# xander683/ConstructionScenePoseEstimation

Measured on AMD Instinct MI355X. Metric: annotated frames/sec (RGB+seg+2D kpts) at 1920×1080, 1/2/4/8 MI355X, higher is better.
Workload: dtype f32

## Files before the change

constructionsceneposeestimation_amd/csrc/csg_kernels.hip:

```cpp
#include <math.h>

#include <algorithm>

#include <type_traits>

#include "csg_crops.h"
#include "csg_kernels.h"
#include "csg_raster_math.h"

namespace csg {

#ifndef CSG_ABLATION
#define CSG_ABLATION 0
#endif
#define DBG(d) (CSG_ABLATION ? (d) : 0u)

constexpr uint64_t kEmptyKey = ~0ull;

__device__ __forceinline__ uint32_t fbits(float f) { return __float_as_uint(f); }

template <int Ctrl, int RowMask, int BankMask>
__device__ __forceinline__ uint32_t dpp_add(uint32_t v) {
  return v + (uint32_t)__builtin_amdgcn_update_dpp(0, (int)v, Ctrl, RowMask, BankMask, false);
}
// ... 891 lines not shown
        } else {
          for (uint32_t d = (ex2 >> 5) + 1u; d <= (e_end >> 5); ++d) L.before[d] = (uint16_t)(ci + 1u);
        }
      }
      __syncthreads();
      for (uint32_t j = tid; j < ((DBG(b.dbg) & 8u) ? 0u : tot2); j += kRB) {
        if (DBG(b.dbg) & 512u) {
          const uint64_t m = __ballot(1);
          if ((uint32_t)__lane_id() == (uint32_t)__ffsll((unsigned long long)m) - 1u) {
            atomicAdd(&b.overflow[14], 1u);
            atomicAdd(&b.overflow[15], (uint32_t)__popcll(m));
          }
        }
        const uint32_t w = L.starts[j >> 5], nb = L.before[j >> 5];
        const uint32_t rank = nb + (uint32_t)__popc(w & (0xFFFFFFFFu >> (31u - (j & 31u))));
        const uint32_t spj = L.span[rank - 1u];
        fragment<kCov>(c, L.img, (int)(spj & 255u), (int)(j + (uint32_t)kTileW - (spj >> 16)), (int)((spj >> 8) & 255u));
      }
      __syncthreads();
    }
  }
}

struct ShadeEntry {
  float P[16];
  int32_t label;
  int32_t tex;
  uint32_t base;
  uint32_t q01, q2;
  uint32_t n01, n2;
};

__device__ __forceinline__ void shade_setup(const SceneDev& s, const BatchDev& b, uint32_t f, uint32_t uid,
                                            ShadeEntry& e) {
  const uint32_t i = uid >> s.uid_shift, g = uid & ((1u << s.uid_shift) - 1u);
  const uint32_t set = b.fset[f];
  const float* tp = s.tri_pos + (size_t)g * 9;
  float p[9];
#pragma unroll
  for (int z = 0; z < 9; ++z) p[z] = tp[z];
  const InstSetDev is = b.iset[(size_t)set * s.n_inst + i];
  e.label = is.label;
  const int tex = is.tex;
  e.tex = tex;
  e.base = is.base;
  const float* tu = s.tri_uv + (size_t)g * 6;
#pragma unroll
  for (int z = 0; z < 6; ++z) e.P[10 + z] = tex >= 0 ? tu[z] : 0.0f;
  bool facing = false;
  if (tex >= 0 || b.depth || b.points || b.normals) {
    Cv3 v[3];
    const float* Cm = b.clip + ((size_t)f * s.n_inst + i) * 12;
#pragma unroll
    for (int z = 0; z < 3; ++z) {
      v[z].x = dot4(Cm + 0, p[3 * z], p[3 * z + 1], p[3 * z + 2]);
      v[z].y = dot4(Cm + 4, p[3 * z], p[3 * z + 1], p[3 * z + 2]);
      v[z].w = dot4(Cm + 8, p[3 * z], p[3 * z + 1], p[3 * z + 2]);
    }
    Hom h;
    hom_setup(v, h);
#pragma unroll
    for (int z = 0; z < 3; ++z) { e.P[z] = h.A[z]; e.P[3 + z] = h.B[z]; e.P[6 + z] = h.C[z]; }
    e.P[9] = h.invdet;
    facing = h.invdet < 0.0f;
  }
  float e1[3], e2[3];
  {
    const float* M = b.models + ((size_t)set * s.n_inst + i) * 16;
#pragma unroll
    for (int r = 0; r < 3; ++r) {
      const float w0 = dot4(M + 4 * r, p[0], p[1], p[2]);
      const float w1 = dot4(M + 4 * r, p[3], p[4], p[5]);
      const float w2 = dot4(M + 4 * r, p[6], p[7], p[8]);
      e1[r] = w1 - w0;
      e2[r] = w2 - w0;
    }
  }
  const float nx = e1[1] * e2[2] - e1[2] * e2[1];
  const float ny = e1[2] * e2[0] - e1[0] * e2[2];
  const float nz = e1[0] * e2[1] - e1[1] * e2[0];
  const float nn = (nx * nx + ny * ny) + nz * nz;
  const LightDev& L = b.lights[set];
  float cs = 0.0f;
  uint32_t n01 = 0, n2 = 0;
  if (nn > 0.0f) {
    const float len = sqrtf(nn);
    const float d = (nx * L.sun_dir[0] + ny * L.sun_dir[1]) + nz * L.sun_dir[2];
    cs = fabsf(d / len);
    if (b.normals) {
      const float sg = facing ? 1.0f : -1.0f;
      n01 = half_bits(sg * (nx / len)) | (half_bits(sg * (ny / len)) << 16);
      n2 = half_bits(sg * (nz / len));
    }
  }
  e.n01 = n01;
  e.n2 = n2;
  uint32_t q[3];
#pragma unroll
  for (int z = 0; z < 3; ++z) {
    const float shade = L.ambient[z] + L.sun[z] * cs;
    const int qq = (int)(shade * 256.0f + 0.5f);
    q[z] = (uint32_t)min(max(qq, 0), 65535);
  }
  e.q01 = q[0] | (q[1] << 16);
  e.q2 = q[2];
  __asm__ volatile("" ::: "memory");
  float P[16];
#pragma unroll
  for (int z = 0; z < 16; ++z) P[z] = e.P[z];
  float D[3], U[3], V[3];
  depth_plane(P, P + 3, P + 6, P[9], D);
  uv_planes(P, P + 3, P + 6, P[9], P + 10, U, V);
#pragma unroll
  for (int z = 0; z < 3; ++z) { e.P[z] = D[z]; e.P[4 + 2 * z] = U[z]; e.P[5 + 2 * z] = V[z]; }
}

__device__ __forceinline__ void shade_pixel(const SceneDev& s, const ShadeEntry& e, int px, int py, bool need_depth,
                                            uint32_t& rgb_out, int32_t& id_out, float& depth_out) {
  const bool textured = e.tex >= 0 && !(DBG(s.dbg) & 4096u);
  const float fx = (float)px + 0.5f, fy = (float)py + 0.5f;
  float r = INFINITY;
  if (need_depth || textured) r = rcp_ieee(plane_at(e.P[0], e.P[1], e.P[2], fx, fy));
  depth_out = need_depth ? r : INFINITY;
  id_out = e.label;
  int base[3] = {(int)(e.base & 255u), (int)((e.base >> 8) & 255u), (int)((e.base >> 16) & 255u)};
  int alb[3];
  if (textured) {
    const f32x2 p0 = {e.P[4], e.P[5]}, p1 = {e.P[6], e.P[7]}, p2 = {e.P[8], e.P[9]};
    const f32x2 uv = ((p0 * fx + p1 * fy) + p2) * r;
    int c[4];
    tex_sample(s, e.tex, uv.x, uv.y, c);
#pragma unroll
    for (int z = 0; z < 3; ++z) alb[z] = div255(__umul24((uint32_t)c[z], (uint32_t)base[z]) + 127u);
  } else {
#pragma unroll
    for (int z = 0; z < 3; ++z) alb[z] = base[z];
  }
  const int q[3] = {(int)(e.q01 & 0xFFFFu), (int)(e.q01 >> 16), (int)e.q2};
  uint32_t o = 0;
#pragma unroll
  for (int z = 0; z < 3; ++z) o |= (uint32_t)min((int)((__umul24((uint32_t)alb[z], (uint32_t)q[z]) + 128u) >> 8), 255) << (8 * z);
  rgb_out = o;
}

#ifndef CSG_VEC_OUT
#define CSG_VEC_OUT 1
#endif
#ifndef CSG_VEC_DEP_ONCE
#define CSG_VEC_DEP_ONCE 1
#endif

#ifndef CSG_SHADE_SLOTS
#define CSG_SHADE_SLOTS (kRasterBlock >= 256 ? 116 : 64)
#endif
constexpr uint32_t kShadeSlots = CSG_SHADE_SLOTS;
static_assert(kShadeSlots <= (uint32_t)kRasterBlock && kShadeSlots < 255u, "one setup thread per slot; 8-bit slot ids");
constexpr int kShadeProbes = 16;
struct ResolveLds {
  uint32_t keys[kShadeSlots];
  uint32_t more;
  ShadeEntry tab[kShadeSlots];
  uint32_t lstat[2 + kColWords][kMaxLdsLabels];
};

constexpr size_t lds_budget(int waves) {
  return kRasterBlock == 256
             ? (waves >= 8 ? 20480u : waves == 7 ? 22528u : waves == 6 ? 26700u : waves == 5 ? 32256u : 40960u)
             : ((157696u / (size_t)(waves * 4 / (kRasterBlock / 64))) & ~511u);
}
static_assert((sizeof(RasterLds<kStage>) > sizeof(ResolveLds) ? sizeof(RasterLds<kStage>) : sizeof(ResolveLds)) +
                      kTilePix * 8 <= lds_budget(CSG_WAVES),
              "k_raster LDS must allow CSG_WAVES workgroups per CU");

template <bool kCov>
struct RasterSide {
  RasterLds<kStageOf<kCov>> r;
};
template <>
struct RasterSide<true> {
  RasterLds<kStageOf<true>> r;
  CovLds cov;
  int32_t rlabel[kStageOf<true>];
};
static_assert((sizeof(RasterSide<true>) > sizeof(ResolveLds) ? sizeof(RasterSide<true>) : sizeof(ResolveLds)) +
                      kTilePix * 8 <= lds_budget(CSG_COV_WAVES),
              "k_raster<true> LDS must allow CSG_COV_WAVES workgroups per CU");

__device__ __forceinline__ int shade_slot(uint32_t* keys, uint32_t uid) {
  const uint32_t h = __umulhi(uid * 2654435761u, kShadeSlots);
#pragma clang loop vectorize(disable) unroll(disable)
  for (int p = 0; p < kShadeProbes; ++p) {
    uint32_t idx = h + (uint32_t)p;
    idx = idx >= kShadeSlots ? idx - kShadeSlots : idx;
    const uint32_t prev = atomicCAS(&keys[idx], kNoAlpha, uid);
    if (prev == kNoAlpha || prev == uid) return (int)idx;
  }
  return -1;
}

#ifndef CSG_SQ_X
#define CSG_SQ_X 2
#endif
#ifndef CSG_SQ_Y
#define CSG_SQ_Y 2
#endif
constexpr uint32_t kSqX = CSG_SQ_X, kSqY = CSG_SQ_Y;
constexpr uint32_t kSqN = kSqX * kSqY;
// ... 17 lines not shown
#endif
#ifndef CSG_NT_RGB
#define CSG_NT_RGB 1
#endif
typedef uint32_t v3u32 __attribute__((ext_vector_type(3)));
typedef float v4f32 __attribute__((ext_vector_type(4)));
typedef uint32_t v2u32 __attribute__((ext_vector_type(2)));
__device__ __forceinline__ void out_f4(float* p, float a, float b2, float c, float d) {
  const v4f32 w = {a, b2, c, d};
  if (CSG_NT_OUT) __builtin_nontemporal_store(w, reinterpret_cast<v4f32*>(p));
  else *reinterpret_cast<v4f32*>(p) = w;
}
__device__ __forceinline__ void out_u2(uint16_t* p, uint32_t a, uint32_t b2) {
  const v2u32 w = {a, b2};
  if (CSG_NT_OUT) __builtin_nontemporal_store(w, reinterpret_cast<v2u32*>(p));
  else *reinterpret_cast<v2u32*>(p) = w;
}
__device__ __forceinline__ void out_rgb4(uint8_t* p, uint32_t c0, uint32_t c1, uint32_t c2, uint32_t c3) {
  const v3u32 w = {c0 | (c1 << 24), (c1 >> 8) | (c2 << 16), (c2 >> 16) | (c3 << 8)};
  if (CSG_NT_RGB) __builtin_nontemporal_store(w, reinterpret_cast<v3u32*>(p));
  else *reinterpret_cast<v3u32*>(p) = w;
}

__device__ __forceinline__ void empty_tile(const SceneDev& s, const BatchDev& b, uint32_t f, uint32_t tile, int ox,
                                           int oy) {
  const int tid = threadIdx.x;
  if (b.n_kp && ((b.kp_tiles[(size_t)f * b.tile_words + (tile >> 5)] >> (tile & 31u)) & 1u)) {
    for (uint32_t k = tid; k < b.n_kp; k += kRB) {
      const size_t o = (size_t)f * b.n_kp + k;
      const uint32_t pp = b.kp_pix[o];
      const int px = (int)(pp & 0xFFFFu) - ox, py = (int)(pp >> 16) - oy;
      if (pp == 0xFFFFFFFFu || px < 0 || px >= kTileW || py < 0 || py >= kTileH) continue;
      b.kp_vis[o] = (b.kp_w[o] <= INFINITY) ? 2 : 1;
    }
  }
  const int ly = tid / (kTileW / 4), lx0 = (tid % (kTileW / 4)) * 4;
  const int py = oy + ly, px0 = ox + lx0;
  if (py >= (int)s.H) return;
  const size_t o = (size_t)f * s.W * s.H + (size_t)py * s.W + px0;
  const uint32_t sky = b.lights[b.fset[f]].sky & 0xFFFFFFu;
  const float nan = __builtin_nanf("");
  if (px0 + 3 < (int)s.W && ((o + b.px_align) & 3u) == 0) {
    if (b.inst) out_ids(b.inst + o, make_int4(-1, -1, -1, -1));
    if (b.rgb) out_rgb4(b.rgb + o * 3, sky, sky, sky, sky);
    if (b.depth) out_f4(b.depth + o, INFINITY, INFINITY, INFINITY, INFINITY);
    if (b.normals) {
      for (int w = 0; w < 3; ++w) out_u2(b.normals + o * 3 + 4 * w, 0u, 0u);
    }
    if (b.points) {
      for (int w = 0; w < 3; ++w) out_f4(b.points + o * 3 + 4 * w, nan, nan, nan, nan);
    }
  } else {
    for (int k = 0; k < 4 && px0 + k < (int)s.W; ++k) {
      if (b.inst) b.inst[o + k] = -1;
      if (b.rgb) {
        b.rgb[(o + k) * 3 + 0] = (uint8_t)(sky & 255u);
        b.rgb[(o + k) * 3 + 1] = (uint8_t)((sky >> 8) & 255u);
        b.rgb[(o + k) * 3 + 2] = (uint8_t)((sky >> 16) & 255u);
      }
      if (b.depth) b.depth[o + k] = INFINITY;
      if (b.normals) b.normals[(o + k) * 3 + 0] = b.normals[(o + k) * 3 + 1] = b.normals[(o + k) * 3 + 2] = 0;
      if (b.points) b.points[(o + k) * 3 + 0] = b.points[(o + k) * 3 + 1] = b.points[(o + k) * 3 + 2] = nan;
    }
  }
}

template <bool kCov>
__global__ __launch_bounds__(kRasterBlock) CSG_RASTER_ATTR void k_raster(SceneDev s, BatchDev b) {
  __shared__ unsigned long long zb[kTilePix];
  constexpr int NS = kStageOf<kCov>;
  __shared__ union Lds {
    RasterSide<kCov> ra;
    ResolveLds q;
  } L;
  const int tid = threadIdx.x;
  uint32_t tile;
  if (!swizzled_tile(blockIdx.x, s.tiles_x, s.tiles_y, tile)) return;
  const uint32_t f = blockIdx.y;
  const int ox = (int)(tile % s.tiles_x) * kTileW, oy = (int)(tile / s.tiles_x) * kTileH;
  const uint32_t* toff = b.tile_off + (size_t)f * (s.n_tiles + 1);
  const Slab sb = b.slab[f];
  const uint32_t beg = min(toff[tile], sb.bin_cap);
  const uint32_t end = (DBG(b.dbg) & 2u) ? beg : min(toff[tile + 1], sb.bin_cap);
  if (beg == end && !(DBG(b.dbg) & 2u)) {
    empty_tile(s, b, f, tile, ox, oy);
    return;
  }
  const uint32_t* bins = b.bins + sb.bin_base;
  const uint32_t rfirst = (CSG_PREFETCH_BIN && tid < NS && beg + (uint32_t)tid < end) ? bins[beg + tid] : 0xFFFFFFFFu;
  for (int p = tid; p < kTilePix; p += kRB) zb[p] = kEmptyKey;
  CovLds* covp = nullptr;
  int32_t* rlabel = nullptr;
  if constexpr (kCov) {
    covp = &L.ra.cov;
    rlabel = L.ra.rlabel;
    CovLds& covl = *covp;
    for (int p = tid; p < kCovSlots * (kTilePix / 32); p += kRB) (&covl.mask[0][0])[p] = 0u;
    if (tid < kCovSlots) covl.keys[tid] = kNoAlpha;
    if (tid == 0) covl.ovf = 0u;
  }
  const Rec* recs = b.recs + sb.rec_base;
  RasterCtx c{s.aquad, s.acls, zb, ox, oy, s.inv_near, s.inv_far, b.dbg, b.overflow, covp, rlabel,
              kCov ? b.covered + (size_t)f * b.n_labels : nullptr};
  __syncthreads();
  raster_block<kCov, NS>(c, s, b, L.ra.r, beg, end, bins, recs, sb.rec_cap, rfirst);
  __syncthreads();
  if constexpr (kCov) {
    const CovLds& covl = *covp;
// ... 9 lines not shown
    if ((tid % kTPS) == 0 && lab != kNoAlpha) {
      if (covl.ovf) atomicOr(&c.gcov[lab], kCovUnknown);
      else atomicAdd(&c.gcov[lab], n);
    }
    __syncthreads();
  }

  if (DBG(b.dbg) & 1u) {
    if (tid == 0 && zb[0] == 0ull && b.inst) b.inst[0] = 0;
    return;
  }
  if (b.n_kp && ((b.kp_tiles[(size_t)f * b.tile_words + (tile >> 5)] >> (tile & 31u)) & 1u)) {
    for (uint32_t k = tid; k < b.n_kp; k += kRB) {
      const size_t o = (size_t)f * b.n_kp + k;
      const uint32_t pp = b.kp_pix[o];
      const int px = (int)(pp & 0xFFFFu) - ox, py = (int)(pp >> 16) - oy;
      if (pp == 0xFFFFFFFFu || px < 0 || px >= kTileW || py < 0 || py >= kTileH) continue;
      const unsigned long long key = zb[zb_index(px, py)];
      const float d = key == kEmptyKey ? INFINITY : rcp_ieee(__uint_as_float(0xFFFFFFFFu - (uint32_t)(key >> 32)));
      b.kp_vis[o] = (b.kp_w[o] <= d) ? 2 : 1;
    }
    __syncthreads();
  }
  const bool want_stats = b.stats != nullptr;
  const uint32_t nl = want_stats ? min(b.n_labels, (uint32_t)kMaxLdsLabels) : 0u;
  uint32_t (*lstat)[kMaxLdsLabels] = L.q.lstat;
  for (uint32_t l = tid; l < nl; l += kRB) {
#pragma unroll
    for (int w = 0; w < 2 + kColWords; ++w) lstat[w][l] = 0;
  }
  const int ly = tid / (kTileW / 4), lx0 = (tid % (kTileW / 4)) * 4;
  const int py = oy + ly;
  const bool row_ok = py < (int)s.H;
  const int px0 = ox + lx0;
  unsigned long long* zrow = &zb[zb_index(lx0, ly) & ~3];
  const int zsw = CSG_ZB_SWIZZLE ? (ly & 3) : 0;
  auto zpix = [&](int k) -> unsigned long long& { return zrow[k ^ zsw]; };
  uint32_t pend = 0;
  uint32_t inmask = 0;
  __shared__ uint32_t drw[2][kRB / 64];
  {
    const uint32_t sky = b.lights[b.fset[f]].sky & 0xFFFFFFu;
    const unsigned long long bgword = (unsigned long long)sky | (0xFFFFFFFFull << 32);
    uint32_t kmn = 0xFFFFFFFFu, kmx = 0u;
#pragma unroll
    for (int k = 0; k < 4; ++k) {
      const bool in = row_ok && px0 + k < (int)s.W;
      inmask |= in ? 1u << k : 0u;
      const unsigned long long key = zpix(k);
      if (in && key != kEmptyKey) {
        pend |= 1u << k;
        kmn = min(kmn, (uint32_t)(key >> 32));
        kmx = max(kmx, (uint32_t)(key >> 32));
      } else {
        zpix(k) = bgword;
      }
    }
    if (b.drange) {
#pragma unroll
      for (int o = 32; o > 0; o >>= 1) {
        kmn = min(kmn, (uint32_t)__shfl_xor((int)kmn, o, 64));
        kmx = max(kmx, (uint32_t)__shfl_xor((int)kmx, o, 64));
      }
      if ((tid & 63) == 0) { drw[0][tid >> 6] = kmn; drw[1][tid >> 6] = kmx; }
    }
  }
  const size_t npx = (size_t)s.W * s.H;
  const size_t o = (size_t)f * npx + (size_t)py * s.W + px0;
  const uint32_t bgmask = inmask & ~pend;
  const bool need_depth = b.depth || b.points;
  auto round = [&](const bool first) __attribute__((always_inline)) -> bool {
    if ((uint32_t)tid < kShadeSlots) L.q.keys[tid] = kNoAlpha;
    __syncthreads();
    if (tid == 0) L.q.more = 0;
    if (first && b.drange && tid == 0) {
      uint32_t kmn = drw[0][0], kmx = drw[1][0];
#pragma unroll
      for (int w = 1; w < kRB / 64; ++w) { kmn = min(kmn, drw[0][w]); kmx = max(kmx, drw[1][w]); }
      if (kmn <= kmx) {
        const float dmin = rcp_ieee(__uint_as_float(0xFFFFFFFFu - kmn));
        const float dmax = rcp_ieee(__uint_as_float(0xFFFFFFFFu - kmx));
        if (__float_as_uint(dmin) < b.drange[f]) atomicMin(&b.drange[f], __float_as_uint(dmin));
        if (__float_as_uint(dmax) > b.drange[b.drange_F + f]) atomicMax(&b.drange[b.drange_F + f], __float_as_uint(dmax));
      }
    }
    uint32_t slots = 0xFFFFFFFFu;
    {
      uint32_t prev_uid = 0xFFFFFFFFu, prev_slot = 0xFFu;
#pragma unroll
      for (int k = 0; k < 4; ++k) {
        if ((pend >> k) & 1u) {
          const uint32_t uid = (uint32_t)zpix(k);
          uint32_t sl;
          if (uid == prev_uid) sl = prev_slot;
          else {
            const int r = shade_slot(L.q.keys, uid);
            sl = r < 0 ? 0xFFu : (uint32_t)r;
          }
          prev_uid = uid;
          prev_slot = sl;
          slots = (slots & ~(0xFFu << (8 * k))) | (sl << (8 * k));
        } else {
          prev_uid = 0xFFFFFFFFu;
        }
      }
    }
    __syncthreads();
    {
      const uint32_t u = (uint32_t)tid < kShadeSlots ? L.q.keys[tid] : kNoAlpha;
      if (u != kNoAlpha) {
        ShadeEntry& e = L.q.tab[tid];
        if (DBG(b.dbg) & 8192u) {
          e = ShadeEntry{};
          e.P[2] = 1.0f; e.tex = -1; e.label = 0;
        } else {
          shade_setup(s, b, f, u, e);
        }
      }
    }
    __syncthreads();
    if (row_ok) {
      int qx0 = px0, qy = py;
      asm volatile("" : "+v"(qx0), "+v"(qy));
      const size_t qo = (size_t)f * npx + (size_t)qy * s.W + qx0;
      int32_t run = -1;
      uint32_t cnt = 0, xmin = 0, xmax = 0;
      auto flush_run = [&]() {
        if (DBG(b.dbg) & 16384u) return;
        if (run >= 0 && (uint32_t)run < nl) {
          const uint32_t col = xmin - (uint32_t)ox;
          atomicAdd(&lstat[0][run], cnt);
          atomicOr(&lstat[2 + (kColWords > 1 ? col >> 5 : 0u)][run], (0xFu >> (3u - (xmax - xmin))) << (col & 31u));
          atomicOr(&lstat[1][run], 1u << ((uint32_t)qy - (uint32_t)oy));
        } else if (run >= 0 && b.stats && (uint32_t)run < b.n_labels) {
          uint32_t* st = b.stats + ((size_t)f * b.n_labels + (uint32_t)run) * 5;
          atomicAdd(&st[0], cnt);
          atomicMin(&st[1], xmin);
          atomicMin(&st[2], (uint32_t)qy);
          atomicMax(&st[3], xmax);
          atomicMax(&st[4], (uint32_t)qy);
        }
      };
      bool vec = false;
      if (CSG_VEC_OUT && (b.depth || b.normals || b.points) && inmask == 0xFu && ((qo + b.px_align) & 3u) == 0) {
        uint32_t done = first ? bgmask : 0u;
#pragma unroll
        for (int k = 0; k < 4; ++k) done |= ((slots >> (8 * k)) & 0xFFu) != 0xFFu ? 1u << k : 0u;
        vec = done == 0xFu;
      }
#pragma unroll
      for (int k = 0; k < 4; ++k) {
        const int px = qx0 + k;
        const uint32_t sl = (slots >> (8 * k)) & 0xFFu;
        const bool bg = first && ((bgmask >> k) & 1u);
        if (sl == 0xFFu && !bg) continue;
        float dep = INFINITY;
        uint32_t n01 = 0, n2 = 0;
        if (!bg) {
          const ShadeEntry& e = L.q.tab[sl];
          uint32_t rgb;
          int32_t id;
          shade_pixel(s, e, px, qy, need_depth && !(CSG_VEC_DEP_ONCE && vec), rgb, id, dep);
          n01 = e.n01;
          n2 = e.n2;
          zpix(k) = (unsigned long long)rgb | ((unsigned long long)(uint32_t)id << 32);
          pend &= ~(1u << k);
          if (want_stats) {
            if (id != run) {
              flush_run();
              run = id;
              cnt = 0;
              xmin = (uint32_t)px;
            }
            ++cnt;
            xmax = (uint32_t)px;
          }
        }
        if (vec) continue;
        if (b.depth) b.depth[qo + k] = dep;
        if (b.normals) {
          uint16_t* d = b.normals + (qo + k) * 3;
          d[0] = (uint16_t)(n01 & 0xFFFFu);
          d[1] = (uint16_t)(n01 >> 16);
          d[2] = (uint16_t)n2;
        }
        if (b.points) {
          float pt[3];
          if (bg) pt[0] = pt[1] = pt[2] = __builtin_nanf("");
          else unproject(b.cam + (size_t)f * kCamFloats, px, qy, dep, pt);
          float* d = b.points + (qo + k) * 3;
          d[0] = pt[0];
          d[1] = pt[1];
          d[2] = pt[2];
        }
      }
      flush_run();
      if (vec) {
        const uint32_t bgv = first ? bgmask : 0u;
        float dv[4];
#pragma unroll
        for (int k = 0; k < 4; ++k) {
          const ShadeEntry& e = L.q.tab[(bgv >> k) & 1u ? 0u : (slots >> (8 * k)) & 0xFFu];
          const float fx = (float)(qx0 + k) + 0.5f, fy = (float)qy + 0.5f;
          dv[k] = ((bgv >> k) & 1u) || !need_depth ? INFINITY : rcp_ieee(plane_at(e.P[0], e.P[1], e.P[2], fx, fy));
        }
        if (b.depth) out_f4(b.depth + qo, dv[0], dv[1], dv[2], dv[3]);
        if (b.normals) {
          uint32_t n01[4], n2[4];
#pragma unroll
          for (int k = 0; k < 4; ++k) {
            const bool bg = (bgv >> k) & 1u;
            const ShadeEntry& e = L.q.tab[bg ? 0u : (slots >> (8 * k)) & 0xFFu];
            n01[k] = bg ? 0u : e.n01;
            n2[k] = bg ? 0u : e.n2;
          }
          uint16_t* d = b.normals + qo * 3;
          out_u2(d, n01[0], n2[0] | (n01[1] << 16));
          out_u2(d + 4, (n01[1] >> 16) | (n2[1] << 16), n01[2]);
          out_u2(d + 8, n2[2] | (n01[3] << 16), (n01[3] >> 16) | (n2[3] << 16));
        }
        if (b.points) {
          float pt[12];
#pragma unroll
          for (int k = 0; k < 4; ++k) {
            if ((bgv >> k) & 1u) pt[3 * k] = pt[3 * k + 1] = pt[3 * k + 2] = __builtin_nanf("");
            else unproject(b.cam + (size_t)f * kCamFloats, qx0 + k, qy, dv[k], pt + 3 * k);
          }
          float* d = b.points + qo * 3;
          out_f4(d, pt[0], pt[1], pt[2], pt[3]);
          out_f4(d + 4, pt[4], pt[5], pt[6], pt[7]);
          out_f4(d + 8, pt[8], pt[9], pt[10], pt[11]);
        }
      }
    }
    if (pend) L.q.more = 1;
    __syncthreads();
    return L.q.more != 0;
  };
  if (round(true)) {
#pragma clang loop unroll(disable)
    while (round(false)) {
    }
  }
  if (row_ok) {
    uint32_t rgb[4];
    int32_t ids[4];
#pragma unroll
    for (int k = 0; k < 4; ++k) {
      const unsigned long long w = zpix(k);
      rgb[k] = (uint32_t)w;
      ids[k] = (int32_t)(w >> 32);
    }
    if (px0 + 3 < (int)s.W && ((o + b.px_align) & 3u) == 0) {
      if (b.inst) out_ids(b.inst + o, make_int4(ids[0], ids[1], ids[2], ids[3]));
      if (b.rgb) out_rgb4(b.rgb + o * 3, rgb[0], rgb[1], rgb[2], rgb[3]);
    } else {
      for (int k = 0; k < 4 && px0 + k < (int)s.W; ++k) {
        if (b.inst) b.inst[o + k] = ids[k];
        if (b.rgb) {
          b.rgb[(o + k) * 3 + 0] = (uint8_t)(rgb[k] & 255u);
          b.rgb[(o + k) * 3 + 1] = (uint8_t)((rgb[k] >> 8) & 255u);
          b.rgb[(o + k) * 3 + 2] = (uint8_t)((rgb[k] >> 16) & 255u);
        }
      }
    }
  }
  if (b.stats) {
    __syncthreads();
    uint32_t* st = b.stats + (size_t)f * b.n_labels * 5;
    for (uint32_t l = tid; l < nl; l += kRB) {
      const uint32_t cnt = lstat[0][l];
      if (cnt) {
        const uint32_t rm = lstat[1][l];
        uint32_t cm = lstat[2][l], cm_hi = cm, lo_w = 0, hi_w = 0;
#pragma unroll
        for (int w = 1; w < kColWords; ++w) {
          const uint32_t m = lstat[2 + w][l];
          if (!cm && m) { cm = m; lo_w = (uint32_t)w; }
          if (m) { cm_hi = m; hi_w = (uint32_t)w; }
        }
        if (!cm_hi) cm_hi = cm;
        atomicAdd(&st[l * 5 + 0], cnt);
        atomicMin(&st[l * 5 + 1], (uint32_t)ox + 32u * lo_w + (uint32_t)(__ffs(cm) - 1));
        atomicMin(&st[l * 5 + 2], (uint32_t)oy + (uint32_t)(__ffs(rm) - 1));
        atomicMax(&st[l * 5 + 3], (uint32_t)ox + 32u * hi_w + 31u - (uint32_t)__clz(cm_hi));
        atomicMax(&st[l * 5 + 4], (uint32_t)oy + 31u - (uint32_t)__clz(rm));
      }
    }
  }
}

__global__ void k_init_stats(uint32_t* st, uint32_t n) {
  const uint32_t k = blockIdx.x * blockDim.x + threadIdx.x;
  if (k < n) {
    const uint32_t c = k % 5;
    st[k] = (c == 1 || c == 2) ? 0xFFFFFFFFu : 0u;
  }
}

__device__ __forceinline__ void project_one(const float* pv, const float* p, float Wf, float Hf, float nearc,
                                            float& u, float& v, int& vis, int& px, int& py) {
  const float X = dot4(pv + 0, p[0], p[1], p[2]);
  const float Y = dot4(pv + 4, p[0], p[1], p[2]);
  const float Wc = dot4(pv + 8, p[0], p[1], p[2]);
  px = py = -1;
  if (!(Wc >= nearc)) {
    u = -1.0f; v = -1.0f; vis = 0;
    return;
  }
// ... 227 lines not shown
                 uint64_t bin_pool, int use_hints, Slab* slab, uint64_t* need, hipStream_t st) {
  hipLaunchKernelGGL(k_plan, dim3(1), dim3(64), 0, st, frames, F, def_rec, def_bin, rec_pool, bin_pool, use_hints,
                     slab, need);
}

void launch_scan(const SceneDev& s, const BatchDev& b, uint32_t F, hipStream_t st) {
  hipLaunchKernelGGL(k_scan, dim3(F), dim3(kBlock), 0, st, s, b);
}

void launch_bin(const SceneDev& s, const BatchDev& b, uint32_t F, uint32_t blocks, hipStream_t st) {
  dim3 g(blocks, F);
  const uint32_t band = s.n_tiles < kBinBand ? s.n_tiles : kBinBand;
  if (s.n_tiles > kBinBand) hipLaunchKernelGGL(k_bin<true>, g, dim3(kBlock), band * sizeof(uint32_t), st, s, b);
  else hipLaunchKernelGGL(k_bin<false>, g, dim3(kBlock), band * sizeof(uint32_t), st, s, b);
}

void launch_colscan(const SceneDev& s, const BatchDev& b, uint32_t F, hipStream_t st) {
  hipLaunchKernelGGL(k_colscan, dim3((s.n_tiles + kBlock - 1) / kBlock, F), dim3(kBlock), 0, st, s, b);
}

void launch_raster(const SceneDev& s, const BatchDev& b, uint32_t F, hipStream_t st) {
  const uint32_t squares = ((s.tiles_x + kSqX - 1) / kSqX) * ((s.tiles_y + kSqY - 1) / kSqY);
  dim3 g(8 * kSqN * ((squares + 7) / 8), F);
  if (b.covered) hipLaunchKernelGGL(k_raster<true>, g, dim3(kRasterBlock), 0, st, s, b);
  else hipLaunchKernelGGL(k_raster<false>, g, dim3(kRasterBlock), 0, st, s, b);
}

void launch_init_stats(const BatchDev& b, uint32_t F, hipStream_t st) {
  const uint32_t n = F * b.n_labels * 5;
  if (!n || !b.stats) return;
  hipLaunchKernelGGL(k_init_stats, dim3((n + 255) / 256), dim3(256), 0, st, b.stats, n);
}

void launch_keypoints(const SceneDev& s, const BatchDev& b, uint32_t F, hipStream_t st) {
  if (!b.n_kp) return;
  dim3 g((b.n_kp + 255) / 256, F);
  hipLaunchKernelGGL(k_keypoints, g, dim3(256), 0, st, s, b);
}

void launch_inst_bounds(const SceneDev& s, const Chunk* chunks, uint32_t n_chunks, const float* models,
                        uint32_t* out, hipStream_t st) {
  hipLaunchKernelGGL(k_inst_bounds, dim3(n_chunks), dim3(kBlock), 0, st, s, chunks, models, out);
}

void launch_project(const float* pts, uint32_t n, const float* pv12, float W, float H, float near_clip, float* uv,
                    int32_t* vis, hipStream_t st) {
  hipLaunchKernelGGL(k_project, dim3((n + 255) / 256), dim3(256), 0, st, pts, n, pv12, W, H, near_clip, uv, vis);
}
// ... 269 lines not shown
```

Baseline: 25750.

## Add lean raster kernel specialization for RGB+seg-only outputs

Adds a compile-time kLean variant of k_raster that is chosen when depth, normals, points, stats and drange are all disabled. The variant removes normal and depth plane handling, label-stat LDS tables and depth-range reductions, and shrinks the shade entry and resolve LDS. It also recomputes per-thread pixel coordinates from tid at several points, so fewer values stay live in registers and occupancy can rise. The cost is a third kernel instantiation, more code to maintain, and a little extra index arithmetic.

```diff
diff --git a/constructionsceneposeestimation_amd/csrc/csg_kernels.hip b/constructionsceneposeestimation_amd/csrc/csg_kernels.hip
--- a/constructionsceneposeestimation_amd/csrc/csg_kernels.hip
+++ b/constructionsceneposeestimation_amd/csrc/csg_kernels.hip
@@ -937,6 +937,7 @@
   }
 }
 
+template <bool kLean>
 struct ShadeEntry {
   float P[16];
   int32_t label;
@@ -945,9 +946,24 @@
   uint32_t q01, q2;
   uint32_t n01, n2;
 };
-
+template <>
+struct ShadeEntry<true> {
+  float P[16];
+  int32_t label;
+  int32_t tex;
+  uint32_t base;
+  uint32_t q01, q2;
+};
+template <bool kLean>
+struct SetupOpt {
+  bool facing = false;
+};
+template <>
+struct SetupOpt<true> {};
+
+template <bool kLean>
 __device__ __forceinline__ void shade_setup(const SceneDev& s, const BatchDev& b, uint32_t f, uint32_t uid,
-                                            ShadeEntry& e) {
+                                            ShadeEntry<kLean>& e) {
   const uint32_t i = uid >> s.uid_shift, g = uid & ((1u << s.uid_shift) - 1u);
   const uint32_t set = b.fset[f];
   const float* tp = s.tri_pos + (size_t)g * 9;
@@ -962,8 +978,8 @@
   const float* tu = s.tri_uv + (size_t)g * 6;
 #pragma unroll
   for (int z = 0; z < 6; ++z) e.P[10 + z] = tex >= 0 ? tu[z] : 0.0f;
-  bool facing = false;
-  if (tex >= 0 || b.depth || b.points || b.normals) {
+  SetupOpt<kLean> opt;
+  if (tex >= 0 || (!kLean && (b.depth || b.points || b.normals))) {
     Cv3 v[3];
     const float* Cm = b.clip + ((size_t)f * s.n_inst + i) * 12;
 #pragma unroll
@@ -977,7 +993,7 @@
 #pragma unroll
     for (int z = 0; z < 3; ++z) { e.P[z] = h.A[z]; e.P[3 + z] = h.B[z]; e.P[6 + z] = h.C[z]; }
     e.P[9] = h.invdet;
-    facing = h.invdet < 0.0f;
+    if constexpr (!kLean) opt.facing = h.invdet < 0.0f;
   }
   float e1[3], e2[3];
   {
@@ -997,19 +1013,27 @@
   const float nn = (nx * nx + ny * ny) + nz * nz;
   const LightDev& L = b.lights[set];
   float cs = 0.0f;
-  uint32_t n01 = 0, n2 = 0;
-  if (nn > 0.0f) {
-    const float len = sqrtf(nn);
-    const float d = (nx * L.sun_dir[0] + ny * L.sun_dir[1]) + nz * L.sun_dir[2];
-    cs = fabsf(d / len);
-    if (b.normals) {
-      const float sg = facing ? 1.0f : -1.0f;
-      n01 = half_bits(sg * (nx / len)) | (half_bits(sg * (ny / len)) << 16);
-      n2 = half_bits(sg * (nz / len));
-    }
-  }
-  e.n01 = n01;
-  e.n2 = n2;
+  if constexpr (kLean) {
+    if (nn > 0.0f) {
+      const float len = sqrtf(nn);
+      const float d = (nx * L.sun_dir[0] + ny * L.sun_dir[1]) + nz * L.sun_dir[2];
+      cs = fabsf(d / len);
+    }
+  } else {
+    uint32_t n01 = 0, n2 = 0;
+    if (nn > 0.0f) {
+      const float len = sqrtf(nn);
+      const float d = (nx * L.sun_dir[0] + ny * L.sun_dir[1]) + nz * L.sun_dir[2];
+      cs = fabsf(d / len);
+      if (b.normals) {
+        const float sg = opt.facing ? 1.0f : -1.0f;
+        n01 = half_bits(sg * (nx / len)) | (half_bits(sg * (ny / len)) << 16);
+        n2 = half_bits(sg * (nz / len));
+      }
+    }
+    e.n01 = n01;
+    e.n2 = n2;
+  }
   uint32_t q[3];
 #pragma unroll
   for (int z = 0; z < 3; ++z) {
@@ -1030,13 +1054,18 @@
   for (int z = 0; z < 3; ++z) { e.P[z] = D[z]; e.P[4 + 2 * z] = U[z]; e.P[5 + 2 * z] = V[z]; }
 }
 
-__device__ __forceinline__ void shade_pixel(const SceneDev& s, const ShadeEntry& e, int px, int py, bool need_depth,
-                                            uint32_t& rgb_out, int32_t& id_out, float& depth_out) {
+template <bool kLean>
+__device__ __forceinline__ void shade_pixel(const SceneDev& s, const ShadeEntry<kLean>& e, int px, int py,
+                                            bool need_depth, uint32_t& rgb_out, int32_t& id_out, float& depth_out) {
   const bool textured = e.tex >= 0 && !(DBG(s.dbg) & 4096u);
   const float fx = (float)px + 0.5f, fy = (float)py + 0.5f;
   float r = INFINITY;
-  if (need_depth || textured) r = rcp_ieee(plane_at(e.P[0], e.P[1], e.P[2], fx, fy));
-  depth_out = need_depth ? r : INFINITY;
+  if constexpr (kLean) {
+    if (textured) r = rcp_ieee(plane_at(e.P[0], e.P[1], e.P[2], fx, fy));
+  } else {
+    if (need_depth || textured) r = rcp_ieee(plane_at(e.P[0], e.P[1], e.P[2], fx, fy));
+    depth_out = need_depth ? r : INFINITY;
+  }
   id_out = e.label;
   int base[3] = {(int)(e.base & 255u), (int)((e.base >> 8) & 255u), (int)((e.base >> 16) & 255u)};
   int alb[3];
@@ -1071,11 +1100,18 @@
 constexpr uint32_t kShadeSlots = CSG_SHADE_SLOTS;
 static_assert(kShadeSlots <= (uint32_t)kRasterBlock && kShadeSlots < 255u, "one setup thread per slot; 8-bit slot ids");
 constexpr int kShadeProbes = 16;
+template <bool kLean>
 struct ResolveLds {
   uint32_t keys[kShadeSlots];
   uint32_t more;
-  ShadeEntry tab[kShadeSlots];
+  ShadeEntry<false> tab[kShadeSlots];
   uint32_t lstat[2 + kColWords][kMaxLdsLabels];
+};
+template <>
+struct ResolveLds<true> {
+  uint32_t keys[kShadeSlots];
+  uint32_t more;
+  ShadeEntry<true> tab[kShadeSlots];
 };
 
 constexpr size_t lds_budget(int waves) {
@@ -1083,7 +1119,7 @@
              ? (waves >= 8 ? 20480u : waves == 7 ? 22528u : waves == 6 ? 26700u : waves == 5 ? 32256u : 40960u)
              : ((157696u / (size_t)(waves * 4 / (kRasterBlock / 64))) & ~511u);
 }
-static_assert((sizeof(RasterLds<kStage>) > sizeof(ResolveLds) ? sizeof(RasterLds<kStage>) : sizeof(ResolveLds)) +
+static_assert((sizeof(RasterLds<kStage>) > sizeof(ResolveLds<false>) ? sizeof(RasterLds<kStage>) : sizeof(ResolveLds<false>)) +
                       kTilePix * 8 <= lds_budget(CSG_WAVES),
               "k_raster LDS must allow CSG_WAVES workgroups per CU");
 
@@ -1097,7 +1133,7 @@
   CovLds cov;
   int32_t rlabel[kStageOf<true>];
 };
-static_assert((sizeof(RasterSide<true>) > sizeof(ResolveLds) ? sizeof(RasterSide<true>) : sizeof(ResolveLds)) +
+static_assert((sizeof(RasterSide<true>) > sizeof(ResolveLds<false>) ? sizeof(RasterSide<true>) : sizeof(ResolveLds<false>)) +
                       kTilePix * 8 <= lds_budget(CSG_COV_WAVES),
               "k_raster<true> LDS must allow CSG_COV_WAVES workgroups per CU");
 
@@ -1161,6 +1197,7 @@
   else *reinterpret_cast<v3u32*>(p) = w;
 }
 
+template <bool kLean>
 __device__ __forceinline__ void empty_tile(const SceneDev& s, const BatchDev& b, uint32_t f, uint32_t tile, int ox,
                                            int oy) {
   const int tid = threadIdx.x;
@@ -1178,16 +1215,18 @@
   if (py >= (int)s.H) return;
   const size_t o = (size_t)f * s.W * s.H + (size_t)py * s.W + px0;
   const uint32_t sky = b.lights[b.fset[f]].sky & 0xFFFFFFu;
-  const float nan = __builtin_nanf("");
+  [[maybe_unused]] const float nan = __builtin_nanf("");
   if (px0 + 3 < (int)s.W && ((o + b.px_align) & 3u) == 0) {
     if (b.inst) out_ids(b.inst + o, make_int4(-1, -1, -1, -1));
     if (b.rgb) out_rgb4(b.rgb + o * 3, sky, sky, sky, sky);
-    if (b.depth) out_f4(b.depth + o, INFINITY, INFINITY, INFINITY, INFINITY);
-    if (b.normals) {
-      for (int w = 0; w < 3; ++w) out_u2(b.normals + o * 3 + 4 * w, 0u, 0u);
-    }
-    if (b.points) {
-      for (int w = 0; w < 3; ++w) out_f4(b.points + o * 3 + 4 * w, nan, nan, nan, nan);
+    if constexpr (!kLean) {
+      if (b.depth) out_f4(b.depth + o, INFINITY, INFINITY, INFINITY, INFINITY);
+      if (b.normals) {
+        for (int w = 0; w < 3; ++w) out_u2(b.normals + o * 3 + 4 * w, 0u, 0u);
+      }
+      if (b.points) {
+        for (int w = 0; w < 3; ++w) out_f4(b.points + o * 3 + 4 * w, nan, nan, nan, nan);
+      }
     }
   } else {
     for (int k = 0; k < 4 && px0 + k < (int)s.W; ++k) {
@@ -1197,20 +1236,40 @@
         b.rgb[(o + k) * 3 + 1] = (uint8_t)((sky >> 8) & 255u);
         b.rgb[(o + k) * 3 + 2] = (uint8_t)((sky >> 16) & 255u);
       }
-      if (b.depth) b.depth[o + k] = INFINITY;
-      if (b.normals) b.normals[(o + k) * 3 + 0] = b.normals[(o + k) * 3 + 1] = b.normals[(o + k) * 3 + 2] = 0;
-      if (b.points) b.points[(o + k) * 3 + 0] = b.points[(o + k) * 3 + 1] = b.points[(o + k) * 3 + 2] = nan;
-    }
-  }
-}
-
-template <bool kCov>
+      if constexpr (!kLean) {
+        if (b.depth) b.depth[o + k] = INFINITY;
+        if (b.normals) b.normals[(o + k) * 3 + 0] = b.normals[(o + k) * 3 + 1] = b.normals[(o + k) * 3 + 2] = 0;
+        if (b.points) b.points[(o + k) * 3 + 0] = b.points[(o + k) * 3 + 1] = b.points[(o + k) * 3 + 2] = nan;
+      }
+    }
+  }
+}
+
+__device__ __forceinline__ uint32_t (*drange_lds())[kRasterBlock / 64] {
+  __shared__ uint32_t drw[2][kRasterBlock / 64];
+  return drw;
+}
+template <bool kLean>
+struct ResolveOpt {
+  bool want_stats, need_depth;
+  uint32_t nl;
+  uint32_t (*lstat)[kMaxLdsLabels];
+  uint32_t (*drw)[kRasterBlock / 64];
+};
+template <>
+struct ResolveOpt<true> {};
+
+#ifndef CSG_RASTER_LEAN
+#define CSG_RASTER_LEAN 1
+#endif
+template <bool kCov, bool kLean>
 __global__ __launch_bounds__(kRasterBlock) CSG_RASTER_ATTR void k_raster(SceneDev s, BatchDev b) {
+  static_assert(!(kCov && kLean), "the coverage kernel is general");
   __shared__ unsigned long long zb[kTilePix];
   constexpr int NS = kStageOf<kCov>;
   __shared__ union Lds {
     RasterSide<kCov> ra;
-    ResolveLds q;
+    ResolveLds<kLean> q;
   } L;
   const int tid = threadIdx.x;
   uint32_t tile;
@@ -1222,7 +1281,7 @@
   const uint32_t beg = min(toff[tile], sb.bin_cap);
   const uint32_t end = (DBG(b.dbg) & 2u) ? beg : min(toff[tile + 1], sb.bin_cap);
   if (beg == end && !(DBG(b.dbg) & 2u)) {
-    empty_tile(s, b, f, tile, ox, oy);
+    empty_tile<kLean>(s, b, f, tile, ox, oy);
     return;
   }
   const uint32_t* bins = b.bins + sb.bin_base;
@@ -1278,27 +1337,39 @@
     }
     __syncthreads();
   }
-  const bool want_stats = b.stats != nullptr;
-  const uint32_t nl = want_stats ? min(b.n_labels, (uint32_t)kMaxLdsLabels) : 0u;
-  uint32_t (*lstat)[kMaxLdsLabels] = L.q.lstat;
-  for (uint32_t l = tid; l < nl; l += kRB) {
-#pragma unroll
-    for (int w = 0; w < 2 + kColWords; ++w) lstat[w][l] = 0;
+  ResolveOpt<kLean> opt;
+  if constexpr (!kLean) {
+    opt.want_stats = b.stats != nullptr;
+    opt.nl = opt.want_stats ? min(b.n_labels, (uint32_t)kMaxLdsLabels) : 0u;
+    opt.lstat = L.q.lstat;
+    opt.drw = drange_lds();
+    for (uint32_t l = tid; l < opt.nl; l += kRB) {
+#pragma unroll
+      for (int w = 0; w < 2 + kColWords; ++w) opt.lstat[w][l] = 0;
+    }
   }
   const int ly = tid / (kTileW / 4), lx0 = (tid % (kTileW / 4)) * 4;
   const int py = oy + ly;
   const bool row_ok = py < (int)s.H;
   const int px0 = ox + lx0;
   unsigned long long* zrow = &zb[zb_index(lx0, ly) & ~3];
-  const int zsw = CSG_ZB_SWIZZLE ? (ly & 3) : 0;
+  int zsw = CSG_ZB_SWIZZLE ? (ly & 3) : 0;
   auto zpix = [&](int k) -> unsigned long long& { return zrow[k ^ zsw]; };
+  auto zfresh = [&]() __attribute__((always_inline)) {
+    if constexpr (kLean) {
+      int t = tid;
+      asm volatile("" : "+v"(t));
+      const int y = t / (kTileW / 4), x0 = (t % (kTileW / 4)) * 4;
+      zrow = &zb[zb_index(x0, y) & ~3];
+      zsw = CSG_ZB_SWIZZLE ? (y & 3) : 0;
+    }
+  };
   uint32_t pend = 0;
   uint32_t inmask = 0;
-  __shared__ uint32_t drw[2][kRB / 64];
   {
     const uint32_t sky = b.lights[b.fset[f]].sky & 0xFFFFFFu;
     const unsigned long long bgword = (unsigned long long)sky | (0xFFFFFFFFull << 32);
-    uint32_t kmn = 0xFFFFFFFFu, kmx = 0u;
+    [[maybe_unused]] uint32_t kmn = 0xFFFFFFFFu, kmx = 0u;
 #pragma unroll
     for (int k = 0; k < 4; ++k) {
       const bool in = row_ok && px0 + k < (int)s.W;
@@ -1306,41 +1377,48 @@
       const unsigned long long key = zpix(k);
       if (in && key != kEmptyKey) {
         pend |= 1u << k;
-        kmn = min(kmn, (uint32_t)(key >> 32));
-        kmx = max(kmx, (uint32_t)(key >> 32));
+        if constexpr (!kLean) {
+          kmn = min(kmn, (uint32_t)(key >> 32));
+          kmx = max(kmx, (uint32_t)(key >> 32));
+        }
       } else {
         zpix(k) = bgword;
       }
     }
-    if (b.drange) {
-#pragma unroll
-      for (int o = 32; o > 0; o >>= 1) {
-        kmn = min(kmn, (uint32_t)__shfl_xor((int)kmn, o, 64));
-        kmx = max(kmx, (uint32_t)__shfl_xor((int)kmx, o, 64));
-      }
-      if ((tid & 63) == 0) { drw[0][tid >> 6] = kmn; drw[1][tid >> 6] = kmx; }
+    if constexpr (!kLean) {
+      if (b.drange) {
+#pragma unroll
+        for (int o = 32; o > 0; o >>= 1) {
+          kmn = min(kmn, (uint32_t)__shfl_xor((int)kmn, o, 64));
+          kmx = max(kmx, (uint32_t)__shfl_xor((int)kmx, o, 64));
+        }
+        if ((tid & 63) == 0) { opt.drw[0][tid >> 6] = kmn; opt.drw[1][tid >> 6] = kmx; }
+      }
     }
   }
   const size_t npx = (size_t)s.W * s.H;
   const size_t o = (size_t)f * npx + (size_t)py * s.W + px0;
-  const uint32_t bgmask = inmask & ~pend;
-  const bool need_depth = b.depth || b.points;
+  [[maybe_unused]] const uint32_t bgmask = inmask & ~pend;
+  if constexpr (!kLean) opt.need_depth = b.depth || b.points;
   auto round = [&](const bool first) __attribute__((always_inline)) -> bool {
     if ((uint32_t)tid < kShadeSlots) L.q.keys[tid] = kNoAlpha;
     __syncthreads();
     if (tid == 0) L.q.more = 0;
-    if (first && b.drange && tid == 0) {
-      uint32_t kmn = drw[0][0], kmx = drw[1][0];
-#pragma unroll
-      for (int w = 1; w < kRB / 64; ++w) { kmn = min(kmn, drw[0][w]); kmx = max(kmx, drw[1][w]); }
-      if (kmn <= kmx) {
-        const float dmin = rcp_ieee(__uint_as_float(0xFFFFFFFFu - kmn));
-        const float dmax = rcp_ieee(__uint_as_float(0xFFFFFFFFu - kmx));
-        if (__float_as_uint(dmin) < b.drange[f]) atomicMin(&b.drange[f], __float_as_uint(dmin));
-        if (__float_as_uint(dmax) > b.drange[b.drange_F + f]) atomicMax(&b.drange[b.drange_F + f], __float_as_uint(dmax));
+    if constexpr (!kLean) {
+      if (first && b.drange && tid == 0) {
+        uint32_t kmn = opt.drw[0][0], kmx = opt.drw[1][0];
+#pragma unroll
+        for (int w = 1; w < kRB / 64; ++w) { kmn = min(kmn, opt.drw[0][w]); kmx = max(kmx, opt.drw[1][w]); }
+        if (kmn <= kmx) {
+          const float dmin = rcp_ieee(__uint_as_float(0xFFFFFFFFu - kmn));
+          const float dmax = rcp_ieee(__uint_as_float(0xFFFFFFFFu - kmx));
+          if (__float_as_uint(dmin) < b.drange[f]) atomicMin(&b.drange[f], __float_as_uint(dmin));
+          if (__float_as_uint(dmax) > b.drange[b.drange_F + f]) atomicMax(&b.drange[b.drange_F + f], __float_as_uint(dmax));
+        }
       }
     }
     uint32_t slots = 0xFFFFFFFFu;
+    zfresh();
     {
       uint32_t prev_uid = 0xFFFFFFFFu, prev_slot = 0xFFu;
 #pragma unroll
@@ -1365,127 +1443,151 @@
     {
       const uint32_t u = (uint32_t)tid < kShadeSlots ? L.q.keys[tid] : kNoAlpha;
       if (u != kNoAlpha) {
-        ShadeEntry& e = L.q.tab[tid];
+        ShadeEntry<kLean>& e = L.q.tab[tid];
         if (DBG(b.dbg) & 8192u) {
-          e = ShadeEntry{};
+          e = ShadeEntry<kLean>{};
           e.P[2] = 1.0f; e.tex = -1; e.label = 0;
         } else {
-          shade_setup(s, b, f, u, e);
+          shade_setup<kLean>(s, b, f, u, e);
         }
       }
     }
     __syncthreads();
     if (row_ok) {
       int qx0 = px0, qy = py;
-      asm volatile("" : "+v"(qx0), "+v"(qy));
-      const size_t qo = (size_t)f * npx + (size_t)qy * s.W + qx0;
-      int32_t run = -1;
-      uint32_t cnt = 0, xmin = 0, xmax = 0;
-      auto flush_run = [&]() {
-        if (DBG(b.dbg) & 16384u) return;
-        if (run >= 0 && (uint32_t)run < nl) {
-          const uint32_t col = xmin - (uint32_t)ox;
-          atomicAdd(&lstat[0][run], cnt);
-          atomicOr(&lstat[2 + (kColWords > 1 ? col >> 5 : 0u)][run], (0xFu >> (3u - (xmax - xmin))) << (col & 31u));
-          atomicOr(&lstat[1][run], 1u << ((uint32_t)qy - (uint32_t)oy));
-        } else if (run >= 0 && b.stats && (uint32_t)run < b.n_labels) {
-          uint32_t* st = b.stats + ((size_t)f * b.n_labels + (uint32_t)run) * 5;
-          atomicAdd(&st[0], cnt);
-          atomicMin(&st[1], xmin);
-          atomicMin(&st[2], (uint32_t)qy);
-          atomicMax(&st[3], xmax);
-          atomicMax(&st[4], (uint32_t)qy);
-        }
-      };
-      bool vec = false;
-      if (CSG_VEC_OUT && (b.depth || b.normals || b.points) && inmask == 0xFu && ((qo + b.px_align) & 3u) == 0) {
-        uint32_t done = first ? bgmask : 0u;
-#pragma unroll
-        for (int k = 0; k < 4; ++k) done |= ((slots >> (8 * k)) & 0xFFu) != 0xFFu ? 1u << k : 0u;
-        vec = done == 0xFu;
-      }
-#pragma unroll
-      for (int k = 0; k < 4; ++k) {
-        const int px = qx0 + k;
-        const uint32_t sl = (slots >> (8 * k)) & 0xFFu;
-        const bool bg = first && ((bgmask >> k) & 1u);
-        if (sl == 0xFFu && !bg) continue;
-        float dep = INFINITY;
-        uint32_t n01 = 0, n2 = 0;
-        if (!bg) {
-          const ShadeEntry& e = L.q.tab[sl];
+      if constexpr (kLean) {
+        int t = tid;
+        asm volatile("" : "+v"(t));
+        qx0 = ox + (t % (kTileW / 4)) * 4;
+        qy = oy + t / (kTileW / 4);
+        zfresh();
+      } else {
+        asm volatile("" : "+v"(qx0), "+v"(qy));
+      }
+      if constexpr (kLean) {
+#pragma unroll
+        for (int k = 0; k < 4; ++k) {
+          const int px = qx0 + k;
+          const uint32_t sl = (slots >> (8 * k)) & 0xFFu;
+          if (sl == 0xFFu) continue;
+          const ShadeEntry<true>& e = L.q.tab[sl];
           uint32_t rgb;
           int32_t id;
-          shade_pixel(s, e, px, qy, need_depth && !(CSG_VEC_DEP_ONCE && vec), rgb, id, dep);
-          n01 = e.n01;
-          n2 = e.n2;
+          float dep;
+          shade_pixel<true>(s, e, px, qy, false, rgb, id, dep);
           zpix(k) = (unsigned long long)rgb | ((unsigned long long)(uint32_t)id << 32);
           pend &= ~(1u << k);
-          if (want_stats) {
-            if (id != run) {
-              flush_run();
-              run = id;
-              cnt = 0;
-              xmin = (uint32_t)px;
+        }
+      } else {
+        const size_t qo = (size_t)f * npx + (size_t)qy * s.W + qx0;
+        int32_t run = -1;
+        uint32_t cnt = 0, xmin = 0, xmax = 0;
+        auto flush_run = [&]() {
+          if (DBG(b.dbg) & 16384u) return;
+          if (run >= 0 && (uint32_t)run < opt.nl) {
+            const uint32_t col = xmin - (uint32_t)ox;
+            atomicAdd(&opt.lstat[0][run], cnt);
+            atomicOr(&opt.lstat[2 + (kColWords > 1 ? col >> 5 : 0u)][run], (0xFu >> (3u - (xmax - xmin))) << (col & 31u));
+            atomicOr(&opt.lstat[1][run], 1u << ((uint32_t)qy - (uint32_t)oy));
+          } else if (run >= 0 && b.stats && (uint32_t)run < b.n_labels) {
+            uint32_t* st = b.stats + ((size_t)f * b.n_labels + (uint32_t)run) * 5;
+            atomicAdd(&st[0], cnt);
+            atomicMin(&st[1], xmin);
+            atomicMin(&st[2], (uint32_t)qy);
+            atomicMax(&st[3], xmax);
+            atomicMax(&st[4], (uint32_t)qy);
+          }
+        };
+        bool vec = false;
+        if (CSG_VEC_OUT && (b.depth || b.normals || b.points) && inmask == 0xFu && ((qo + b.px_align) & 3u) == 0) {
+          uint32_t done = first ? bgmask : 0u;
+#pragma unroll
+          for (int k = 0; k < 4; ++k) done |= ((slots >> (8 * k)) & 0xFFu) != 0xFFu ? 1u << k : 0u;
+          vec = done == 0xFu;
+        }
+#pragma unroll
+        for (int k = 0; k < 4; ++k) {
+          const int px = qx0 + k;
+          const uint32_t sl = (slots >> (8 * k)) & 0xFFu;
+          const bool bg = first && ((bgmask >> k) & 1u);
+          if (sl == 0xFFu && !bg) continue;
+          float dep = INFINITY;
+          uint32_t n01 = 0, n2 = 0;
+          if (!bg) {
+            const ShadeEntry<false>& e = L.q.tab[sl];
+            uint32_t rgb;
+            int32_t id;
+            shade_pixel<false>(s, e, px, qy, opt.need_depth && !(CSG_VEC_DEP_ONCE && vec), rgb, id, dep);
+            n01 = e.n01;
+            n2 = e.n2;
+            zpix(k) = (unsigned long long)rgb | ((unsigned long long)(uint32_t)id << 32);
+            pend &= ~(1u << k);
+            if (opt.want_stats) {
+              if (id != run) {
+                flush_run();
+                run = id;
+                cnt = 0;
+                xmin = (uint32_t)px;
+              }
+              ++cnt;
+              xmax = (uint32_t)px;
             }
-            ++cnt;
-            xmax = (uint32_t)px;
+          }
+          if (vec) continue;
+          if (b.depth) b.depth[qo + k] = dep;
+          if (b.normals) {
+            uint16_t* d = b.normals + (qo + k) * 3;
+            d[0] = (uint16_t)(n01 & 0xFFFFu);
+            d[1] = (uint16_t)(n01 >> 16);
+            d[2] = (uint16_t)n2;
+          }
+          if (b.points) {
+            float pt[3];
+            if (bg) pt[0] = pt[1] = pt[2] = __builtin_nanf("");
+            else unproject(b.cam + (size_t)f * kCamFloats, px, qy, dep, pt);
+            float* d = b.points + (qo + k) * 3;
+            d[0] = pt[0];
+            d[1] = pt[1];
+            d[2] = pt[2];
           }
         }
-        if (vec) continue;
-        if (b.depth) b.depth[qo + k] = dep;
-        if (b.normals) {
-          uint16_t* d = b.normals + (qo + k) * 3;
-          d[0] = (uint16_t)(n01 & 0xFFFFu);
-          d[1] = (uint16_t)(n01 >> 16);
-          d[2] = (uint16_t)n2;
-        }
-        if (b.points) {
-          float pt[3];
-          if (bg) pt[0] = pt[1] = pt[2] = __builtin_nanf("");
-          else unproject(b.cam + (size_t)f * kCamFloats, px, qy, dep, pt);
-          float* d = b.points + (qo + k) * 3;
-          d[0] = pt[0];
-          d[1] = pt[1];
-          d[2] = pt[2];
-        }
-      }
-      flush_run();
-      if (vec) {
-        const uint32_t bgv = first ? bgmask : 0u;
-        float dv[4];
-#pragma unroll
-        for (int k = 0; k < 4; ++k) {
-          const ShadeEntry& e = L.q.tab[(bgv >> k) & 1u ? 0u : (slots >> (8 * k)) & 0xFFu];
-          const float fx = (float)(qx0 + k) + 0.5f, fy = (float)qy + 0.5f;
-          dv[k] = ((bgv >> k) & 1u) || !need_depth ? INFINITY : rcp_ieee(plane_at(e.P[0], e.P[1], e.P[2], fx, fy));
-        }
-        if (b.depth) out_f4(b.depth + qo, dv[0], dv[1], dv[2], dv[3]);
-        if (b.normals) {
-          uint32_t n01[4], n2[4];
+        flush_run();
+        if (vec) {
+          const uint32_t bgv = first ? bgmask : 0u;
+          float dv[4];
 #pragma unroll
           for (int k = 0; k < 4; ++k) {
-            const bool bg = (bgv >> k) & 1u;
-            const ShadeEntry& e = L.q.tab[bg ? 0u : (slots >> (8 * k)) & 0xFFu];
-            n01[k] = bg ? 0u : e.n01;
-            n2[k] = bg ? 0u : e.n2;
+            const ShadeEntry<false>& e = L.q.tab[(bgv >> k) & 1u ? 0u : (slots >> (8 * k)) & 0xFFu];
+            const float fx = (float)(qx0 + k) + 0.5f, fy = (float)qy + 0.5f;
+            dv[k] = ((bgv >> k) & 1u) || !opt.need_depth ? INFINITY : rcp_ieee(plane_at(e.P[0], e.P[1], e.P[2], fx, fy));
           }
-          uint16_t* d = b.normals + qo * 3;
-          out_u2(d, n01[0], n2[0] | (n01[1] << 16));
-          out_u2(d + 4, (n01[1] >> 16) | (n2[1] << 16), n01[2]);
-          out_u2(d + 8, n2[2] | (n01[3] << 16), (n01[3] >> 16) | (n2[3] << 16));
-        }
-        if (b.points) {
-          float pt[12];
-#pragma unroll
-          for (int k = 0; k < 4; ++k) {
-            if ((bgv >> k) & 1u) pt[3 * k] = pt[3 * k + 1] = pt[3 * k + 2] = __builtin_nanf("");
-            else unproject(b.cam + (size_t)f * kCamFloats, qx0 + k, qy, dv[k], pt + 3 * k);
+          if (b.depth) out_f4(b.depth + qo, dv[0], dv[1], dv[2], dv[3]);
+          if (b.normals) {
+            uint32_t n01[4], n2[4];
+#pragma unroll
+            for (int k = 0; k < 4; ++k) {
+              const bool bg = (bgv >> k) & 1u;
+              const ShadeEntry<false>& e = L.q.tab[bg ? 0u : (slots >> (8 * k)) & 0xFFu];
+              n01[k] = bg ? 0u : e.n01;
+              n2[k] = bg ? 0u : e.n2;
+            }
+            uint16_t* d = b.normals + qo * 3;
+            out_u2(d, n01[0], n2[0] | (n01[1] << 16));
+            out_u2(d + 4, (n01[1] >> 16) | (n2[1] << 16), n01[2]);
+            out_u2(d + 8, n2[2] | (n01[3] << 16), (n01[3] >> 16) | (n2[3] << 16));
           }
-          float* d = b.points + qo * 3;
-          out_f4(d, pt[0], pt[1], pt[2], pt[3]);
-          out_f4(d + 4, pt[4], pt[5], pt[6], pt[7]);
-          out_f4(d + 8, pt[8], pt[9], pt[10], pt[11]);
+          if (b.points) {
+            float pt[12];
+#pragma unroll
+            for (int k = 0; k < 4; ++k) {
+              if ((bgv >> k) & 1u) pt[3 * k] = pt[3 * k + 1] = pt[3 * k + 2] = __builtin_nanf("");
+              else unproject(b.cam + (size_t)f * kCamFloats, qx0 + k, qy, dv[k], pt + 3 * k);
+            }
+            float* d = b.points + qo * 3;
+            out_f4(d, pt[0], pt[1], pt[2], pt[3]);
+            out_f4(d + 4, pt[4], pt[5], pt[6], pt[7]);
+            out_f4(d + 8, pt[8], pt[9], pt[10], pt[11]);
+          }
         }
       }
     }
@@ -1501,46 +1603,57 @@
   if (row_ok) {
     uint32_t rgb[4];
     int32_t ids[4];
+    zfresh();
 #pragma unroll
     for (int k = 0; k < 4; ++k) {
       const unsigned long long w = zpix(k);
       rgb[k] = (uint32_t)w;
       ids[k] = (int32_t)(w >> 32);
     }
-    if (px0 + 3 < (int)s.W && ((o + b.px_align) & 3u) == 0) {
-      if (b.inst) out_ids(b.inst + o, make_int4(ids[0], ids[1], ids[2], ids[3]));
-      if (b.rgb) out_rgb4(b.rgb + o * 3, rgb[0], rgb[1], rgb[2], rgb[3]);
+    int sx0 = px0;
+    size_t so = o;
+    if constexpr (kLean) {
+      int t = tid;
+      asm volatile("" : "+v"(t));
+      sx0 = ox + (t % (kTileW / 4)) * 4;
+      so = (size_t)f * npx + (size_t)(oy + t / (kTileW / 4)) * s.W + sx0;
+    }
+    if (sx0 + 3 < (int)s.W && ((so + b.px_align) & 3u) == 0) {
+      if (b.inst) out_ids(b.inst + so, make_int4(ids[0], ids[1], ids[2], ids[3]));
+      if (b.rgb) out_rgb4(b.rgb + so * 3, rgb[0], rgb[1], rgb[2], rgb[3]);
     } else {
-      for (int k = 0; k < 4 && px0 + k < (int)s.W; ++k) {
-        if (b.inst) b.inst[o + k] = ids[k];
+      for (int k = 0; k < 4 && sx0 + k < (int)s.W; ++k) {
+        if (b.inst) b.inst[so + k] = ids[k];
         if (b.rgb) {
-          b.rgb[(o + k) * 3 + 0] = (uint8_t)(rgb[k] & 255u);
-          b.rgb[(o + k) * 3 + 1] = (uint8_t)((rgb[k] >> 8) & 255u);
-          b.rgb[(o + k) * 3 + 2] = (uint8_t)((rgb[k] >> 16) & 255u);
+          b.rgb[(so + k) * 3 + 0] = (uint8_t)(rgb[k] & 255u);
+          b.rgb[(so + k) * 3 + 1] = (uint8_t)((rgb[k] >> 8) & 255u);
+          b.rgb[(so + k) * 3 + 2] = (uint8_t)((rgb[k] >> 16) & 255u);
         }
       }
     }
   }
-  if (b.stats) {
-    __syncthreads();
-    uint32_t* st = b.stats + (size_t)f * b.n_labels * 5;
-    for (uint32_t l = tid; l < nl; l += kRB) {
-      const uint32_t cnt = lstat[0][l];
-      if (cnt) {
-        const uint32_t rm = lstat[1][l];
-        uint32_t cm = lstat[2][l], cm_hi = cm, lo_w = 0, hi_w = 0;
-#pragma unroll
-        for (int w = 1; w < kColWords; ++w) {
-          const uint32_t m = lstat[2 + w][l];
-          if (!cm && m) { cm = m; lo_w = (uint32_t)w; }
-          if (m) { cm_hi = m; hi_w = (uint32_t)w; }
+  if constexpr (!kLean) {
+    if (b.stats) {
+      __syncthreads();
+      uint32_t* st = b.stats + (size_t)f * b.n_labels * 5;
+      for (uint32_t l = tid; l < opt.nl; l += kRB) {
+        const uint32_t cnt = opt.lstat[0][l];
+        if (cnt) {
+          const uint32_t rm = opt.lstat[1][l];
+          uint32_t cm = opt.lstat[2][l], cm_hi = cm, lo_w = 0, hi_w = 0;
+#pragma unroll
+          for (int w = 1; w < kColWords; ++w) {
+            const uint32_t m = opt.lstat[2 + w][l];
+            if (!cm && m) { cm = m; lo_w = (uint32_t)w; }
+            if (m) { cm_hi = m; hi_w = (uint32_t)w; }
+          }
+          if (!cm_hi) cm_hi = cm;
+          atomicAdd(&st[l * 5 + 0], cnt);
+          atomicMin(&st[l * 5 + 1], (uint32_t)ox + 32u * lo_w + (uint32_t)(__ffs(cm) - 1));
+          atomicMin(&st[l * 5 + 2], (uint32_t)oy + (uint32_t)(__ffs(rm) - 1));
+          atomicMax(&st[l * 5 + 3], (uint32_t)ox + 32u * hi_w + 31u - (uint32_t)__clz(cm_hi));
+          atomicMax(&st[l * 5 + 4], (uint32_t)oy + 31u - (uint32_t)__clz(rm));
         }
-        if (!cm_hi) cm_hi = cm;
-        atomicAdd(&st[l * 5 + 0], cnt);
-        atomicMin(&st[l * 5 + 1], (uint32_t)ox + 32u * lo_w + (uint32_t)(__ffs(cm) - 1));
-        atomicMin(&st[l * 5 + 2], (uint32_t)oy + (uint32_t)(__ffs(rm) - 1));
-        atomicMax(&st[l * 5 + 3], (uint32_t)ox + 32u * hi_w + 31u - (uint32_t)__clz(cm_hi));
-        atomicMax(&st[l * 5 + 4], (uint32_t)oy + 31u - (uint32_t)__clz(rm));
       }
     }
   }
@@ -1814,8 +1927,10 @@
 void launch_raster(const SceneDev& s, const BatchDev& b, uint32_t F, hipStream_t st) {
   const uint32_t squares = ((s.tiles_x + kSqX - 1) / kSqX) * ((s.tiles_y + kSqY - 1) / kSqY);
   dim3 g(8 * kSqN * ((squares + 7) / 8), F);
-  if (b.covered) hipLaunchKernelGGL(k_raster<true>, g, dim3(kRasterBlock), 0, st, s, b);
-  else hipLaunchKernelGGL(k_raster<false>, g, dim3(kRasterBlock), 0, st, s, b);
+  const bool lean = CSG_RASTER_LEAN && !b.covered && !b.depth && !b.points && !b.normals && !b.stats && !b.drange;
+  if (b.covered) hipLaunchKernelGGL((k_raster<true, false>), g, dim3(kRasterBlock), 0, st, s, b);
+  else if (lean) hipLaunchKernelGGL((k_raster<false, true>), g, dim3(kRasterBlock), 0, st, s, b);
+  else hipLaunchKernelGGL((k_raster<false, false>), g, dim3(kRasterBlock), 0, st, s, b);
 }
 
 void launch_init_stats(const BatchDev& b, uint32_t F, hipStream_t st) {
```

After: 25970 (median of 6 runs). Within noise of the previous version (+0.9%).
